# anton-galkovsky/pointcloudTraj

Measured on AMD Instinct MI355X. Metric: nn_queries_per_sec_10M_point_cloud, higher is better.
Workload: dtype f64; 1 GPU; C3-throughput: 10000000 uniform fp32 points in [0,100.0)^3 (seed 3), 1048576 uniform NN queries per step (4 distinct batches in rotation, seeds [5, 1005, 2005, 3005]), grid kernel, inputs resident in HBM; points_per_gpu=10000000, total_points=10000000, algo=grid, query_batches_in_rotation=4, gpu_work_before_the_warmup_steps=none, full=False, parallelism=single GPU, cards=1

## Files before the change

pointcloudtraj_amd/csrc/kernels.hpp:

```cpp
#pragma once
#include <hip/hip_runtime.h>
#include <stdint.h>
#include <type_traits>

#pragma clang fp contract(off)

#include "bernstein.hpp"
#include "scan.hpp"

namespace pct {

constexpr int kWave = 64;
constexpr uint32_t kNoIndex = 0xFFFFFFFFu;

__device__ __forceinline__ double dist2(double px, double py, double pz, double qx, double qy, double qz)
{
    double dx = px - qx, dy = py - qy, dz = pz - qz;
    double s = dx * dx;
    s = s + dy * dy;
    s = s + dz * dz;
    return s;
}

__device__ __forceinline__ bool better(double d2a, uint32_t ia, double d2b, uint32_t ib)
// ... 1025 lines not shown
}

__device__ __forceinline__ void coop_scan_exact(const float4 *__restrict__ pts, uint32_t s, uint32_t e, uint32_t sub, double qx,
                                                double qy, double qz, double &bd, uint32_t &bi)
{
    for (uint32_t p = s + sub; p < e; p += kCoop) {
        const float4 P = pts[p];
        const double d2 = dist2((double)P.x, (double)P.y, (double)P.z, qx, qy, qz);
        const uint32_t id = __float_as_uint(P.w);
        if (better(d2, id, bd, bi)) { bd = d2; bi = id; }
    }
}

template <bool COUNT>
__device__ __forceinline__ void coop_scan_cube_or_shell(const GridDesc &G, const float4 *__restrict__ pts,
                                                        const uint32_t *__restrict__ cell_start, int cx, int cy, int cz, int r,
                                                        bool full, uint32_t sub, double qx, double qy, double qz, double &bd,
                                                        uint32_t &bi, uint32_t &npts, uint32_t &nruns)
{
    const int x0 = max(cx - r, 0), x1 = min(cx + r, G.gx - 1);
    const int y0 = max(cy - r, 0), y1 = min(cy + r, G.gy - 1);
    const int z0 = max(cz - r, 0), z1 = min(cz + r, G.gz - 1);
    for (int zz = z0; zz <= z1; zz++) {
        const bool zface = (zz == cz - r) || (zz == cz + r);
        for (int yy = y0; yy <= y1; yy++) {
            const uint32_t row = cell_lin(G, 0, yy, zz);
            if (full || zface || yy == cy - r || yy == cy + r) {
                const uint32_t s = cell_start[row + x0], e = cell_start[row + x1 + 1];
                if (COUNT && sub == 0) { npts += e - s; nruns += 1; }
                coop_scan_exact(pts, s, e, sub, qx, qy, qz, bd, bi);
            } else {
                if (cx - r >= 0) {
                    const uint32_t s = cell_start[row + cx - r], e = cell_start[row + cx - r + 1];
                    if (COUNT && sub == 0) { npts += e - s; nruns += 1; }
                    coop_scan_exact(pts, s, e, sub, qx, qy, qz, bd, bi);
                }
                if (cx + r <= G.gx - 1) {
                    const uint32_t s = cell_start[row + cx + r], e = cell_start[row + cx + r + 1];
                    if (COUNT && sub == 0) { npts += e - s; nruns += 1; }
                    coop_scan_exact(pts, s, e, sub, qx, qy, qz, bd, bi);
                }
            }
        }
    }
}

template <int NR, int DEPTH, bool TAIL = false, bool NARROW = false>
__device__ __forceinline__ void coop_screen_rows(const float4 *__restrict__ pts, const uint32_t (&rs)[NR], const uint32_t (&re)[NR],
                                                 uint32_t sub, float qxf, float qyf, float qzf, double qx, double qy, double qz,
                                                 double &bd, uint32_t &bi)
{
    float m1 = __builtin_huge_valf(), m2 = __builtin_huge_valf();
    uint32_t p1 = 0;
    float4 P[NR][DEPTH];
#pragma unroll
    for (int k = 0; k < NR; k++) {
        const uint32_t a = rs[k], b = re[k];
        const uint32_t last = b - 1u;
#pragma unroll
        for (int j = 0; j < DEPTH; j++) P[k][j] = ld_at<NARROW>(pts, min(a + sub + kCoop * j, last));
    }
    uint32_t tp = 0;
    bool tail_on = false, tail_loops = false;
    float4 PT = make_float4(0.0f, 0.0f, 0.0f, 0.0f);
    if constexpr (TAIL) {
        constexpr uint32_t kMain = kCoop * DEPTH;
        uint32_t T = 0;
#pragma unroll
        for (int k = 0; k < NR; k++) {
            const uint32_t t = max(re[k] - rs[k], kMain) - kMain;
            tp = sub >= T ? rs[k] + kMain + (sub - T) : tp;
            T += t;
        }
        tail_on = sub < T && T <= (uint32_t)kCoop;
        tail_loops = T > (uint32_t)kCoop;
        const uint32_t a = rs[NR - 1], b = re[NR - 1];
        tp = tail_on ? tp : min(a + sub + kCoop * (DEPTH - 1), b - 1u);
        PT = ld_at<NARROW>(pts, tp);
    }
#pragma unroll
    for (int k = 0; k < NR; k++) {
        const uint32_t a = rs[k], b = re[k];
#pragma unroll
        for (int j = 0; j < DEPTH; j++) {
            const uint32_t p = a + sub + kCoop * j;
            const float dx = P[k][j].x - qxf, dy = P[k][j].y - qyf, dz = P[k][j].z - qzf;
            float d = __builtin_fmaf(dz, dz, __builtin_fmaf(dy, dy, dx * dx));
            d = (p < b) ? d : __builtin_huge_valf();
            const bool lt = d < m1;
            m2 = __builtin_amdgcn_fmed3f(m1, m2, d);
            p1 = lt ? p : p1;
            m1 = fminf(m1, d);
        }
    }
    auto long_row = [&](uint32_t a, uint32_t b) {
        for (uint32_t p = a + kCoop * DEPTH + sub; p < b; p += kCoop) {
            const float4 Pp = ld_at<NARROW>(pts, p);
            const float dx = Pp.x - qxf, dy = Pp.y - qyf, dz = Pp.z - qzf;
            const float d = __builtin_fmaf(dz, dz, __builtin_fmaf(dy, dy, dx * dx));
            const bool lt = d < m1;
            m2 = __builtin_amdgcn_fmed3f(m1, m2, d);
            p1 = lt ? p : p1;
            m1 = fminf(m1, d);
        }
    };
    if constexpr (TAIL) {
        const float dx = PT.x - qxf, dy = PT.y - qyf, dz = PT.z - qzf;
        float d = __builtin_fmaf(dz, dz, __builtin_fmaf(dy, dy, dx * dx));
        d = tail_on ? d : __builtin_huge_valf();
        const bool lt = d < m1;
        m2 = __builtin_amdgcn_fmed3f(m1, m2, d);
        p1 = lt ? tp : p1;
        m1 = fminf(m1, d);
        if (tail_loops) {
#pragma unroll
            for (int k = 0; k < NR; k++) long_row(rs[k], re[k]);
        }
    } else if constexpr (NR <= 4) {
#pragma unroll
        for (int k = 0; k < NR; k++) long_row(rs[k], re[k]);
    } else {
#pragma unroll 1
        for (int k = 0; k < NR; k++) long_row(rs[k], re[k]);
    }
    auto fold = [&](auto off) {
        constexpr int kPat = swz_xor(decltype(off)::value);
        const float o1 = swz_f32<kPat>(m1), o2 = swz_f32<kPat>(m2);
        const uint32_t op = swz_u32<kPat>(p1);
        const bool lt = o1 < m1;
        m2 = fminf(fminf(m2, o2), fmaxf(m1, o1));
        p1 = lt ? op : p1;
        m1 = fminf(m1, o1);
    };
    fold(std::integral_constant<int, 1>{});
    fold(std::integral_constant<int, 2>{});
    fold(std::integral_constant<int, 4>{});
    bd = __builtin_huge_val();
    bi = kNoIndex;
    if (m1 < __builtin_huge_valf() && m2 > m1 * (1.0f + 0x1p-19f) + 0x1p-90f) {
        const float4 W = ld_at<NARROW>(pts, p1);
        bd = dist2((double)W.x, (double)W.y, (double)W.z, qx, qy, qz);
        bi = __float_as_uint(W.w);
    } else {
#pragma unroll 1
        for (int k = 0; k < NR; k++) coop_scan_exact(pts, rs[k], re[k], sub, qx, qy, qz, bd, bi);
        coop_argmin8(bd, bi);
    }
}

template <bool COUNT>
__device__ __forceinline__ void coop_nn_search(const GridDesc &G, const float4 *__restrict__ pts,
                                               const uint32_t *__restrict__ cell_start, float qxf, float qyf, float qzf,
                                               uint32_t sub, double &bd, uint32_t &bi, uint32_t &npts, uint32_t &nruns)
{
    const double qx = (double)qxf, qy = (double)qyf, qz = (double)qzf;
    const int cx = cell_coord(qxf, G.ox, G.inv_h, G.gx);
    const int cy = cell_coord(qyf, G.oy, G.inv_h, G.gy);
    const int cz = cell_coord(qzf, G.oz, G.inv_h, G.gz);
    bd = __builtin_huge_val();
    bi = kNoIndex;
    if (G.octant_first) {
        const float fx = (qxf - G.ox) * G.inv_h - (float)cx, fy = (qyf - G.oy) * G.inv_h - (float)cy, fz = (qzf - G.oz) * G.inv_h - (float)cz;
        const int xa = max(fx < 0.5f ? cx - 1 : cx, 0), xb = min(fx < 0.5f ? cx : cx + 1, G.gx - 1);
        const int ya = max(fy < 0.5f ? cy - 1 : cy, 0), yb = min(fy < 0.5f ? cy : cy + 1, G.gy - 1);
        const int za = max(fz < 0.5f ? cz - 1 : cz, 0), zb = min(fz < 0.5f ? cz : cz + 1, G.gz - 1);
        uint32_t rs[4], re[4];
        {
            const int ri = (int)sub & 3;
            const bool ok = !((ri >> 1) && zb == za) && !((ri & 1) && yb == ya);
            const uint32_t row = cell_lin(G, 0, (ri & 1) ? yb : ya, (ri >> 1) ? zb : za);
            const uint32_t a = cell_start[row + xa], b = cell_start[row + xb + 1];
            const uint32_t my_s = a, my_e = ok ? b : a;
            if (COUNT && sub < 4) { npts += my_e - my_s; nruns += ok ? 1u : 0u; }
#pragma unroll
            for (int k = 0; k < 4; k++) { rs[k] = (uint32_t)__shfl((int)my_s, k, kCoop); re[k] = (uint32_t)__shfl((int)my_e, k, kCoop); }
        }
        coop_screen_rows<4, 2>(pts, rs, re, sub, qxf, qyf, qzf, qx, qy, qz, bd, bi);
        double bound = __builtin_huge_val();
        if (xa > 0) bound = fmin(bound, qx - (G.oxd + (double)xa * G.hd));
        if (xb < G.gx - 1) bound = fmin(bound, (G.oxd + (double)(xb + 1) * G.hd) - qx);
        if (ya > 0) bound = fmin(bound, qy - (G.oyd + (double)ya * G.hd));
        if (yb < G.gy - 1) bound = fmin(bound, (G.oyd + (double)(yb + 1) * G.hd) - qy);
        if (za > 0) bound = fmin(bound, qz - (G.ozd + (double)za * G.hd));
        if (zb < G.gz - 1) bound = fmin(bound, (G.ozd + (double)(zb + 1) * G.hd) - qz);
        if (bound == __builtin_huge_val()) return;
        bound -= G.hd * (1.0 / 256.0);
        if (bound > 0.0 && bd <= bound * bound) return;
    }
    {
        const int x0 = max(cx - 1, 0), x1 = min(cx + 1, G.gx - 1);
        uint32_t my_s = 0, my_e = 0, s8 = 0, e8 = 0;
        {
            const int zz = cz + (int)sub / 3 - 1, yy = cy + (int)sub % 3 - 1;
            const bool ok = zz >= 0 && zz < G.gz && yy >= 0 && yy < G.gy;
            const uint32_t row = ok ? cell_lin(G, 0, yy, zz) : 0u;
            const uint32_t a = cell_start[row + x0], b = cell_start[row + x1 + 1];
            my_s = a;
            my_e = ok ? b : a;
            const int z8 = cz + 1, y8 = cy + 1;
            const bool ok8 = z8 < G.gz && y8 < G.gy;
            const uint32_t row8 = ok8 ? cell_lin(G, 0, y8, z8) : 0u;
            const uint32_t a8 = cell_start[row8 + x0], b8 = cell_start[row8 + x1 + 1];
            s8 = a8;
            e8 = ok8 ? b8 : a8;
            if (COUNT && sub == 0) {
                npts += e8 - s8; nruns += ok8 ? 1u : 0u;
            }
            if (COUNT) {
                npts += my_e - my_s; nruns += ok ? 1u : 0u;
            }
        }
        uint32_t rs[9], re[9];
#pragma unroll
        for (int k = 0; k < 8; k++) { rs[k] = (uint32_t)__shfl((int)my_s, k, kCoop); re[k] = (uint32_t)__shfl((int)my_e, k, kCoop); }
        rs[8] = s8; re[8] = e8;

        coop_screen_rows<9, 1>(pts, rs, re, sub, qxf, qyf, qzf, qx, qy, qz, bd, bi);
    }
    for (int r = 1;; r++) {
        if (r > 1) {
            coop_scan_cube_or_shell<COUNT>(G, pts, cell_start, cx, cy, cz, r, false, sub, qx, qy, qz, bd, bi, npts, nruns);
            coop_argmin8(bd, bi);
        }
        const double bound = cube_bound(G, cx, cy, cz, r, qx, qy, qz);
        if (bound == __builtin_huge_val() || (bound > 0.0 && bd <= bound * bound)) break;
    }
}


__device__ __forceinline__ bool block_leaves_undecided(const GridDesc &G, int cx, int cy, int cz, int xa, int xb, int ya, int yb, int za, int zb,
                                                       float fx, float fy, float fz, double qx, double qy, double qz, double bd)
{
    {
        const float inf = __builtin_huge_valf();
        float bc = inf;
        bc = fminf(bc, xa > 0 ? fx + (float)(cx - xa) : inf);
        bc = fminf(bc, xb < G.gx - 1 ? (float)(xb + 1 - cx) - fx : inf);
        bc = fminf(bc, ya > 0 ? fy + (float)(cy - ya) : inf);
        bc = fminf(bc, yb < G.gy - 1 ? (float)(yb + 1 - cy) - fy : inf);
        bc = fminf(bc, za > 0 ? fz + (float)(cz - za) : inf);
        bc = fminf(bc, zb < G.gz - 1 ? (float)(zb + 1 - cz) - fz : inf);
        if (bc < inf && fmaxf(fmaxf(fabsf(fx), fabsf(fy)), fabsf(fz)) < 2.0f) {
            const double b = (double)((bc - 0.015625f) * (float)G.hd * 0.999999f);
            if (b > 0.0 && bd <= b * b) return false;
        }
    }
    double bound = __builtin_huge_val();
    if (xa > 0) bound = fmin(bound, qx - (G.oxd + (double)xa * G.hd));
    if (xb < G.gx - 1) bound = fmin(bound, (G.oxd + (double)(xb + 1) * G.hd) - qx);
    if (ya > 0) bound = fmin(bound, qy - (G.oyd + (double)ya * G.hd));
    if (yb < G.gy - 1) bound = fmin(bound, (G.oyd + (double)(yb + 1) * G.hd) - qy);
    if (za > 0) bound = fmin(bound, qz - (G.ozd + (double)za * G.hd));
    if (zb < G.gz - 1) bound = fmin(bound, (G.ozd + (double)(zb + 1) * G.hd) - qz);
    if (bound == __builtin_huge_val()) return false;
    bound -= G.hd * (1.0 / 256.0);
    return !(bound > 0.0 && bd <= bound * bound);
}

template <bool COUNT, bool NARROW>
__device__ __forceinline__ bool coop_stage0(const GridDesc &G, const float4 *__restrict__ pts, const uint32_t *__restrict__ cell_start,
                                            float qxf, float qyf, float qzf, uint32_t sub, double &bd, uint32_t &bi, uint32_t &npts,
                                            uint32_t &nruns)
{
    const double qx = (double)qxf, qy = (double)qyf, qz = (double)qzf;
    const int cx = cell_coord(qxf, G.ox, G.inv_h, G.gx);
    const int cy = cell_coord(qyf, G.oy, G.inv_h, G.gy);
    const int cz = cell_coord(qzf, G.oz, G.inv_h, G.gz);
    const float fx = (qxf - G.ox) * G.inv_h - (float)cx, fy = (qyf - G.oy) * G.inv_h - (float)cy, fz = (qzf - G.oz) * G.inv_h - (float)cz;
    const int xa = max(fx < 0.5f ? cx - 1 : cx, 0), xb = min(fx < 0.5f ? cx : cx + 1, G.gx - 1);
    const int ya = max(fy < 0.5f ? cy - 1 : cy, 0), yb = min(fy < 0.5f ? cy : cy + 1, G.gy - 1);
    const int za = max(fz < 0.5f ? cz - 1 : cz, 0), zb = min(fz < 0.5f ? cz : cz + 1, G.gz - 1);
    uint32_t rs[4], re[4];
    if (G.blocks) {
        const uint32_t u = (uint32_t)(fx < 0.5f ? cx : cx + 1), v = (uint32_t)(fy < 0.5f ? cy : cy + 1), w = (uint32_t)(fz < 0.5f ? cz : cz + 1);
        const uint4 *ent = G.blocks + 2u * ((w * ((uint32_t)G.gy + 1u) + v) * ((uint32_t)G.gx + 1u) + u);
        const uint4 S = ent[0], E = ent[1];
        rs[0] = S.x; rs[1] = S.y; rs[2] = S.z; rs[3] = S.w;
        re[0] = E.x; re[1] = E.y; re[2] = E.z; re[3] = E.w;
        if (COUNT && sub < 4) {
            const int ri = (int)sub;
            const bool ok = !((ri >> 1) && zb == za) && !((ri & 1) && yb == ya);
            npts += re[ri] - rs[ri]; nruns += ok ? 1u : 0u;
        }
    } else {
        const int ri = (int)sub & 3;
        const bool ok = !((ri >> 1) && zb == za) && !((ri & 1) && yb == ya);
        const uint32_t row = cell_lin(G, 0, (ri & 1) ? yb : ya, (ri >> 1) ? zb : za);
        const uint32_t a = ld_at<NARROW>(cell_start, row + (uint32_t)xa), b = ld_at<NARROW>(cell_start, row + (uint32_t)xb + 1u);
        const uint32_t my_s = a, my_e = ok ? b : a;
        if (COUNT && sub < 4) { npts += my_e - my_s; nruns += ok ? 1u : 0u; }
        rs[0] = swz_u32<swz_group_lane(0)>(my_s); re[0] = swz_u32<swz_group_lane(0)>(my_e);
        rs[1] = swz_u32<swz_group_lane(1)>(my_s); re[1] = swz_u32<swz_group_lane(1)>(my_e);
        rs[2] = swz_u32<swz_group_lane(2)>(my_s); re[2] = swz_u32<swz_group_lane(2)>(my_e);
        rs[3] = swz_u32<swz_group_lane(3)>(my_s); re[3] = swz_u32<swz_group_lane(3)>(my_e);
    }
    uint32_t pk0 = (uint32_t)xa | ((uint32_t)xb << 10) | ((uint32_t)ya << 20), pk1 = (uint32_t)yb | ((uint32_t)za << 10) | ((uint32_t)zb << 20);
    asm volatile("" : "+v"(pk0), "+v"(pk1));
    coop_screen_rows<4, 2, true, NARROW>(pts, rs, re, sub, qxf, qyf, qzf, qx, qy, qz, bd, bi);
    asm volatile("" : "+v"(pk0), "+v"(pk1));
    return block_leaves_undecided(G, cx, cy, cz, (int)(pk0 & 1023u), (int)((pk0 >> 10) & 1023u), (int)(pk0 >> 20), (int)(pk1 & 1023u),
                                  (int)((pk1 >> 10) & 1023u), (int)(pk1 >> 20), fx, fy, fz, qx, qy, qz, bd);
}

template <bool COUNT>
__device__ __forceinline__ void wave_cube_search(const GridDesc &G, const float4 *__restrict__ pts, const uint32_t *__restrict__ cell_start,
                                                 float qxf, float qyf, float qzf, double &bd, uint32_t &bi, uint32_t &npts, uint32_t &nruns)
{
    const uint32_t lane = threadIdx.x & 63;
    const double qx = (double)qxf, qy = (double)qyf, qz = (double)qzf;
    const int cx = cell_coord(qxf, G.ox, G.inv_h, G.gx);
    const int cy = cell_coord(qyf, G.oy, G.inv_h, G.gy);
    const int cz = cell_coord(qzf, G.oz, G.inv_h, G.gz);
    const int x0 = max(cx - 1, 0), x1 = min(cx + 1, G.gx - 1);
    uint32_t my_s, my_e;
    {
        const int l = lane < 9 ? (int)lane : 0;
        const int zz = cz + l / 3 - 1, yy = cy + l % 3 - 1;
        const bool ok = zz >= 0 && zz < G.gz && yy >= 0 && yy < G.gy;
        const uint32_t row = ok ? cell_lin(G, 0, yy, zz) : 0u;
        const uint32_t a = cell_start[row + x0], b = cell_start[row + x1 + 1];
        my_s = a;
        my_e = ok ? b : a;
        if (COUNT && lane < 9) { npts += my_e - my_s; nruns += ok ? 1u : 0u; }
    }
    uint32_t rs[9], re[9];
#pragma unroll
    for (int k = 0; k < 9; k++) {
        rs[k] = (uint32_t)__builtin_amdgcn_readlane((int)my_s, k);
        re[k] = (uint32_t)__builtin_amdgcn_readlane((int)my_e, k);
    }
    float m1 = __builtin_huge_valf(), m2 = __builtin_huge_valf();
    uint32_t p1 = 0;
    float4 P[9];
#pragma unroll
    for (int k = 0; k < 9; k++) {
        const uint32_t a = rs[k], b = re[k];
        P[k] = pts[min(a + lane, b > a ? b - 1 : 0u)];
    }
#pragma unroll
    for (int k = 0; k < 9; k++) {
        const uint32_t p = rs[k] + lane;
        const float dx = P[k].x - qxf, dy = P[k].y - qyf, dz = P[k].z - qzf;
        float d = __builtin_fmaf(dz, dz, __builtin_fmaf(dy, dy, dx * dx));
        d = (p < re[k]) ? d : __builtin_huge_valf();
        const bool lt = d < m1;
        m2 = lt ? m1 : fminf(m2, d);
        p1 = lt ? p : p1;
        m1 = fminf(m1, d);
    }
#pragma unroll 1
    for (int k = 0; k < 9; k++)
        for (uint32_t p = rs[k] + 64u + lane; p < re[k]; p += 64u) {
            const float4 Pp = pts[p];
            const float dx = Pp.x - qxf, dy = Pp.y - qyf, dz = Pp.z - qzf;
            const float d = __builtin_fmaf(dz, dz, __builtin_fmaf(dy, dy, dx * dx));
            const bool lt = d < m1;
            m2 = lt ? m1 : fminf(m2, d);
            p1 = lt ? p : p1;
            m1 = fminf(m1, d);
        }
#pragma unroll
    for (int off = 1; off < 64; off <<= 1) {
        const float o1 = __shfl_xor(m1, off, kWave), o2 = __shfl_xor(m2, off, kWave);
        const uint32_t op = (uint32_t)__shfl_xor((int)p1, off, kWave);
        const bool lt = o1 < m1;
        m2 = fminf(fminf(m2, o2), lt ? m1 : o1);
        p1 = lt ? op : p1;
        m1 = fminf(m1, o1);
    }
    bd = __builtin_huge_val();
    bi = kNoIndex;
    if (m1 < __builtin_huge_valf() && m2 > m1 * (1.0f + 0x1p-19f) + 0x1p-90f) {
        const float4 W = pts[p1];
        bd = dist2((double)W.x, (double)W.y, (double)W.z, qx, qy, qz);
        bi = __float_as_uint(W.w);
    } else {
#pragma unroll 1
        for (int k = 0; k < 9; k++)
            for (uint32_t p = rs[k] + lane; p < re[k]; p += 64u) {
                const float4 Pp = pts[p];
                const double d2 = dist2((double)Pp.x, (double)Pp.y, (double)Pp.z, qx, qy, qz);
                const uint32_t id = __float_as_uint(Pp.w);
                if (better(d2, id, bd, bi)) { bd = d2; bi = id; }
            }
        wave_argmin(bd, bi);
    }
}

template <bool COUNT>
__device__ __forceinline__ void coop_finish_shells(const GridDesc &G, const float4 *__restrict__ pts, const uint32_t *__restrict__ cell_start,
                                                   float qxf, float qyf, float qzf, uint32_t sub, double &bd, uint32_t &bi, uint32_t &npts,
                                                   uint32_t &nruns)
{
    const double qx = (double)qxf, qy = (double)qyf, qz = (double)qzf;
    const int cx = cell_coord(qxf, G.ox, G.inv_h, G.gx);
    const int cy = cell_coord(qyf, G.oy, G.inv_h, G.gy);
    const int cz = cell_coord(qzf, G.oz, G.inv_h, G.gz);
    for (int r = 1;; r++) {
        if (r > 1) {
            coop_scan_cube_or_shell<COUNT>(G, pts, cell_start, cx, cy, cz, r, false, sub, qx, qy, qz, bd, bi, npts, nruns);
            coop_argmin8(bd, bi);
        }
        const double bound = cube_bound(G, cx, cy, cz, r, qx, qy, qz);
        if (bound == __builtin_huge_val() || (bound > 0.0 && bd <= bound * bound)) break;
    }
}

template <bool COUNT, bool NARROW>
__device__ __forceinline__ void coop_wave_search(const GridDesc &G, const float4 *__restrict__ pts, const uint32_t *__restrict__ cell_start, bool live,
                                                 float qxf, float qyf, float qzf, uint32_t sub, double &bd, uint32_t &bi, uint32_t &npts, uint32_t &nruns)
{
    bd = __builtin_huge_val();
    bi = kNoIndex;
    bool undecided = false;
    if (live) undecided = coop_stage0<COUNT, NARROW>(G, pts, cell_start, qxf, qyf, qzf, sub, bd, bi, npts, nruns);
    unsigned long long todo = __builtin_amdgcn_ballot_w64(undecided && sub == 0);
    while (todo) {
        const int g = __builtin_ctzll(todo);
        todo &= todo - 1;
        const float bx = __uint_as_float((uint32_t)__builtin_amdgcn_readlane((int)__float_as_uint(qxf), g)),
                    by = __uint_as_float((uint32_t)__builtin_amdgcn_readlane((int)__float_as_uint(qyf), g)),
                    bz = __uint_as_float((uint32_t)__builtin_amdgcn_readlane((int)__float_as_uint(qzf), g));
        double cbd;
        uint32_t cbi;
        wave_cube_search<COUNT>(G, pts, cell_start, bx, by, bz, cbd, cbi, npts, nruns);
        if (((threadIdx.x & 63) >> 3) == (uint32_t)(g >> 3)) { bd = cbd; bi = cbi; }
    }
    if (live && undecided) coop_finish_shells<COUNT>(G, pts, cell_start, qxf, qyf, qzf, sub, bd, bi, npts, nruns);
}

template <bool COUNT, bool NARROW>
__global__ __launch_bounds__(256) __attribute__((amdgpu_waves_per_eu(7, 7))) void nn_grid_coop_kernel(GridDesc G, const float4 *__restrict__ pts,
                                                           const uint32_t *__restrict__ cell_start,
                                                           const float *__restrict__ q, uint32_t Q, uint32_t index_base,
                                                           const float4 *__restrict__ qsorted,
                                                           uint32_t *__restrict__ out_idx, double *__restrict__ out_d2,
                                                           WorkCounters *__restrict__ work)
{
    const uint32_t sub = threadIdx.x & (kCoop - 1);
    const uint32_t bslot = qsorted ? xcd_contiguous_block(blockIdx.x, gridDim.x) : blockIdx.x;
    const uint32_t slot = bslot * (256 / kCoop) + (threadIdx.x / kCoop);
    uint32_t npts = 0, nruns = 0;
    if (G.octant_first) {
        const bool live = slot < Q;
        uint32_t t = slot;
        float qxf = 0.0f, qyf = 0.0f, qzf = 0.0f;
        if (live) {
            if (qsorted) {
                const float4 R = ld_at<NARROW>(qsorted, slot);
                qxf = R.x; qyf = R.y; qzf = R.z; t = __float_as_uint(R.w);
            } else {
                qxf = q[3 * t]; qyf = q[3 * t + 1]; qzf = q[3 * t + 2];
            }
        }
        double bd;
        uint32_t bi;
        coop_wave_search<COUNT, NARROW>(G, pts, cell_start, live, qxf, qyf, qzf, sub, bd, bi, npts, nruns);
        if (live && sub == 0) {
            st_at<NARROW>(out_idx, t, reported_index(bd, bi, index_base));
            st_at<NARROW>(out_d2, t, bd);
        }
    } else if (slot < Q) {
        uint32_t t = slot;
        float qxf, qyf, qzf;
        if (qsorted) {
            const float4 R = qsorted[slot];
            qxf = R.x; qyf = R.y; qzf = R.z; t = __float_as_uint(R.w);
        } else {
            qxf = q[3 * t]; qyf = q[3 * t + 1]; qzf = q[3 * t + 2];
        }
        double bd;
        uint32_t bi;
        coop_nn_search<COUNT>(G, pts, cell_start, qxf, qyf, qzf, sub, bd, bi, npts, nruns);
        if (sub == 0) {
            out_idx[t] = reported_index(bd, bi, index_base);
            out_d2[t] = bd;
        }
    }
    if (COUNT) {
        unsigned long long a = npts, b = nruns;
#pragma unroll
        for (int off = 32; off > 0; off >>= 1) {
            a += (unsigned long long)__shfl_xor((long long)a, off, kWave);
            b += (unsigned long long)__shfl_xor((long long)b, off, kWave);
        }
        if ((threadIdx.x & 63) == 0) { WorkCounters *w = work + (blockIdx.x & (kWorkSlots - 1)); atomicAdd(&w->points, a); atomicAdd(&w->cells, b); }
    }
}

struct BallBox { int x0, x1, y0, y1, z0, z1; };

__device__ __forceinline__ void grid_ball_box(const GridDesc &G, float qxf, float qyf, float qzf, float rf, BallBox &B)
{
    const float pad0 = fabsf(rf) + 0.01f * (1.0f / G.inv_h);
    const float padx = pad0 + 0x1p-22f * (fabsf(qxf) + fabsf(rf)), pady = pad0 + 0x1p-22f * (fabsf(qyf) + fabsf(rf)),
                padz = pad0 + 0x1p-22f * (fabsf(qzf) + fabsf(rf));
    const float hx = qxf + padx, hy = qyf + pady, hz = qzf + padz;
    B.x0 = cell_coord(qxf - padx, G.ox, G.inv_h, G.gx); B.x1 = hx == hx ? cell_coord(hx, G.ox, G.inv_h, G.gx) : G.gx - 1;
    B.y0 = cell_coord(qyf - pady, G.oy, G.inv_h, G.gy); B.y1 = hy == hy ? cell_coord(hy, G.oy, G.inv_h, G.gy) : G.gy - 1;
    B.z0 = cell_coord(qzf - padz, G.oz, G.inv_h, G.gz); B.z1 = hz == hz ? cell_coord(hz, G.oz, G.inv_h, G.gz) : G.gz - 1;
}

template <bool COUNT>
__global__ __launch_bounds__(256) void count_grid_coop_kernel(GridDesc G, const float4 *__restrict__ pts,
                                                              const uint32_t *__restrict__ cell_start,
                                                              const float *__restrict__ q, const float *__restrict__ rad, uint32_t Q,
                                                              const float4 *__restrict__ qsorted, uint32_t *__restrict__ count,
                                                              WorkCounters *__restrict__ work)
{
    const uint32_t sub = threadIdx.x & (kCoop - 1);
    const uint32_t bslot = qsorted ? xcd_contiguous_block(blockIdx.x, gridDim.x) : blockIdx.x;
    const uint32_t slot = bslot * (256 / kCoop) + (threadIdx.x / kCoop);
    uint32_t npts = 0, nruns = 0;
    if (slot < Q) {
        uint32_t t = slot;
        float qxf, qyf, qzf;
        if (qsorted) {
            const float4 R = qsorted[slot];
            qxf = R.x; qyf = R.y; qzf = R.z; t = __float_as_uint(R.w);
        } else {
            qxf = q[3 * t]; qyf = q[3 * t + 1]; qzf = q[3 * t + 2];
        }
        const float rf = rad[t];
        const double qx = (double)qxf, qy = (double)qyf, qz = (double)qzf;
        const double r2 = (double)rf * (double)rf;
        BallBox B;
        grid_ball_box(G, qxf, qyf, qzf, rf, B);
        const int x0 = B.x0, x1 = B.x1, y0 = B.y0, z0 = B.z0;
        const int ny = B.y1 - y0 + 1, nrows = ny * (B.z1 - z0 + 1);
        uint32_t c = 0;
        for (int base = 0; base < nrows; base += 16) {
            uint32_t bs[2], be[2];
#pragma unroll
            for (int h = 0; h < 2; h++) {
                const int k = base + 8 * h + (int)sub;
                const bool ok = k < nrows;
                const uint32_t row = ok ? cell_lin(G, 0, y0 + k % ny, z0 + k / ny) : 0u;
                const uint32_t a = cell_start[row + x0], b = cell_start[row + x1 + 1];
                bs[h] = a; be[h] = ok ? b : a;
                if (COUNT) { npts += be[h] - bs[h]; nruns += ok ? 1u : 0u; }
            }
#pragma unroll
            for (int i = 0; i < 8; i++) {
                if (base + 2 * i >= nrows) break;
                uint32_t rs[2], re[2];
#pragma unroll
                for (int j = 0; j < 2; j++) {
                    const int r = 2 * i + j;
                    rs[j] = (uint32_t)__shfl((int)bs[r >> 3], r & 7, kCoop);
                    re[j] = (uint32_t)__shfl((int)be[r >> 3], r & 7, kCoop);
                }
                float4 P[2][4];
#pragma unroll
                for (int j = 0; j < 2; j++) {
                    const uint32_t last = re[j] > rs[j] ? re[j] - 1 : 0u;
#pragma unroll
                    for (int d = 0; d < 4; d++) P[j][d] = pts[min(rs[j] + sub + kCoop * d, last)];
                }
#pragma unroll
                for (int j = 0; j < 2; j++) {
#pragma unroll
                    for (int d = 0; d < 4; d++) {
                        const bool in = rs[j] + sub + kCoop * d < re[j];
                        c += (in && dist2((double)P[j][d].x, (double)P[j][d].y, (double)P[j][d].z, qx, qy, qz) <= r2) ? 1u : 0u;
                    }
                }
#pragma unroll 1
                for (int j = 0; j < 2; j++)
                    for (uint32_t p = rs[j] + 4 * kCoop + sub; p < re[j]; p += kCoop) {
                        const float4 Pp = pts[p];
                        c += dist2((double)Pp.x, (double)Pp.y, (double)Pp.z, qx, qy, qz) <= r2 ? 1u : 0u;
                    }
            }
        }
#pragma unroll
        for (int off = 1; off < kCoop; off <<= 1) c += (uint32_t)__shfl_xor((int)c, off, kWave);
        if (sub == 0) count[t] = c;
    }
    if (COUNT) {
        unsigned long long a = npts, b = nruns;
#pragma unroll
        for (int off = 32; off > 0; off >>= 1) {
            a += (unsigned long long)__shfl_xor((long long)a, off, kWave);
            b += (unsigned long long)__shfl_xor((long long)b, off, kWave);
        }
        if ((threadIdx.x & 63) == 0) { WorkCounters *w = work + (blockIdx.x & (kWorkSlots - 1)); atomicAdd(&w->points, a); atomicAdd(&w->cells, b); }
    }
}

struct ExpressOut { double d2; double radius; uint32_t idx; uint32_t count; };

struct ExpressSignal { uint32_t *counter; uint32_t *seq; uint32_t value; };

__device__ __forceinline__ void express_done(const ExpressSignal &S)
{
    if (!S.seq) return;
    __threadfence_system();
    bool last = gridDim.x == 1;
    if (!last) {
        last = atomicAdd(S.counter, 1u) == gridDim.x - 1;
        if (last) { atomicExch(S.counter, 0u); __threadfence_system(); }
    }
    if (last) __hip_atomic_store(S.seq, S.value, __ATOMIC_RELEASE, __HIP_MEMORY_SCOPE_SYSTEM);
}

__device__ __forceinline__ void express_done_block(const ExpressSignal &S)
{
    if (!S.seq) return;
    __threadfence_system();
    __syncthreads();
    if (threadIdx.x == 0) express_done(S);
}

__global__ __launch_bounds__(256) void import_floats_kernel(const float *__restrict__ h_src, uint32_t n, float *__restrict__ dst)
{
    const uint32_t i = blockIdx.x * blockDim.x + threadIdx.x;
    if (i < n) dst[i] = h_src[i];
}

__global__ __launch_bounds__(256) void export_results_kernel(const uint32_t *__restrict__ idx, const double *__restrict__ d2, uint32_t Q,
                                                             uint32_t *__restrict__ h_idx, double *__restrict__ h_d2, ExpressSignal sig)
{
    const uint32_t i = blockIdx.x * blockDim.x + threadIdx.x;
    if (i < Q) {
        h_idx[i] = idx[i];
        if (d2) h_d2[i] = d2[i];
    }
    express_done_block(sig);
}

__device__ __forceinline__ void tie_merge(double &d, uint32_t &i, uint32_t &c, double od, uint32_t oi, uint32_t oc)
{
    if (od < d) { d = od; i = oi; c = oc; }
    else if (od == d) { c += oc; i = min(i, oi); }
}

__global__ __launch_bounds__(1024) void nn_small_kernel(const float *__restrict__ x, const float *__restrict__ y,
                                                        const float *__restrict__ z, uint32_t n, double qx, double qy, double qz,
                                                        uint32_t index_base, ExpressOut *__restrict__ out, ExpressSignal sig)
{
    double bd = __builtin_huge_val();
    uint32_t bi = kNoIndex, bc = 0;
    for (uint32_t i = threadIdx.x; i < n; i += 1024) {
        const double d2 = dist2((double)x[i], (double)y[i], (double)z[i], qx, qy, qz);
        if (d2 < bd) { bd = d2; bi = i; bc = 1; }
        else if (d2 == bd) bc++;
    }
#pragma unroll
    for (int off = 32; off > 0; off >>= 1) {
        const double od = __shfl_xor(bd, off, kWave);
        const uint32_t oi = (uint32_t)__shfl_xor((int)bi, off, kWave), oc = (uint32_t)__shfl_xor((int)bc, off, kWave);
        tie_merge(bd, bi, bc, od, oi, oc);
    }
    __shared__ double s_d[16];
    __shared__ uint32_t s_i[16], s_c[16];
    if ((threadIdx.x & 63) == 0) { s_d[threadIdx.x >> 6] = bd; s_i[threadIdx.x >> 6] = bi; s_c[threadIdx.x >> 6] = bc; }
    __syncthreads();
    if (threadIdx.x == 0) {
        for (int w = 1; w < 16; w++) tie_merge(bd, bi, bc, s_d[w], s_i[w], s_c[w]);
        out->d2 = bd;
        out->idx = reported_index(bd, bi, index_base);
        out->count = bc;
        express_done(sig);
    }
}

__global__ __launch_bounds__(1024) void radius_small_kernel(const float *__restrict__ x, const float *__restrict__ y,
                                                            const float *__restrict__ z, uint32_t n, double qx, double qy, double qz,
                                                            double r2, uint32_t index_base, uint32_t *__restrict__ ids, uint32_t cap,
                                                            ExpressOut *__restrict__ out, ExpressSignal sig)
{
    __shared__ uint32_t s_n;
    if (threadIdx.x == 0) s_n = 0;
    __syncthreads();
    for (uint32_t i = threadIdx.x; i < n; i += 1024)
        if (dist2((double)x[i], (double)y[i], (double)z[i], qx, qy, qz) <= r2) {
            const uint32_t pos = atomicAdd(&s_n, 1u);
            if (pos < cap) ids[pos] = i + index_base;
        }
    __syncthreads();
    if (threadIdx.x == 0) out->count = s_n;
    express_done_block(sig);
}

__global__ __launch_bounds__(256) void nn_small_batch_kernel(const float *__restrict__ x, const float *__restrict__ y,
                                                             const float *__restrict__ z, uint32_t n,
                                                             const double *__restrict__ q, uint32_t index_base,
                                                             ExpressOut *__restrict__ out, ExpressSignal sig)
{
    __shared__ double s_d[4];
    __shared__ uint32_t s_i[4];
    const double qx = q[3 * blockIdx.x], qy = q[3 * blockIdx.x + 1], qz = q[3 * blockIdx.x + 2];
    double bd = __builtin_huge_val();
    uint32_t bi = kNoIndex;
    for (uint32_t i = threadIdx.x; i < n; i += 256) {
        const double d2 = dist2((double)x[i], (double)y[i], (double)z[i], qx, qy, qz);
        if (d2 < bd) { bd = d2; bi = i; }
    }
    wave_argmin(bd, bi);
    if ((threadIdx.x & 63) == 0) { s_d[threadIdx.x >> 6] = bd; s_i[threadIdx.x >> 6] = bi; }
    __syncthreads();
    if (threadIdx.x == 0) {
        for (int w = 1; w < 4; w++)
            if (better(s_d[w], s_i[w], bd, bi)) { bd = s_d[w]; bi = s_i[w]; }
        out[blockIdx.x].d2 = bd;
        out[blockIdx.x].idx = reported_index(bd, bi, index_base);
        express_done(sig);
    }
}

__global__ __launch_bounds__(256) void radius_small_batch_kernel(const float *__restrict__ x, const float *__restrict__ y,
                                                                 const float *__restrict__ z, uint32_t n,
                                                                 const double *__restrict__ q, const double *__restrict__ r,
                                                                 uint32_t index_base, uint32_t *__restrict__ ids,
                                                                 uint32_t cap_per_query, ExpressOut *__restrict__ out, ExpressSignal sig)
{
    __shared__ uint32_t s_n;
    if (threadIdx.x == 0) s_n = 0;
    __syncthreads();
    const double qx = q[3 * blockIdx.x], qy = q[3 * blockIdx.x + 1], qz = q[3 * blockIdx.x + 2];
    const double r2 = r[blockIdx.x] * r[blockIdx.x];
    for (uint32_t i = threadIdx.x; i < n; i += 256)
        if (dist2((double)x[i], (double)y[i], (double)z[i], qx, qy, qz) <= r2) {
            const uint32_t pos = atomicAdd(&s_n, 1u);
            if (pos < cap_per_query) ids[(size_t)blockIdx.x * cap_per_query + pos] = i + index_base;
        }
    __syncthreads();
    if (threadIdx.x == 0) out[blockIdx.x].count = s_n;
// ... 278 lines not shown
```

Before: 8.243 billion queries/s.

## Seed wave fallback with stage-0 result and scan only reachable remainder cells

```diff
diff --git a/pointcloudtraj_amd/csrc/kernels.hpp b/pointcloudtraj_amd/csrc/kernels.hpp
--- a/pointcloudtraj_amd/csrc/kernels.hpp
+++ b/pointcloudtraj_amd/csrc/kernels.hpp
@@ -1351,88 +1351,105 @@
                                   (int)((pk1 >> 10) & 1023u), (int)(pk1 >> 20), fx, fy, fz, qx, qy, qz, bd);
 }
 
+constexpr int kRemRows = 4;
 template <bool COUNT>
-__device__ __forceinline__ void wave_cube_search(const GridDesc &G, const float4 *__restrict__ pts, const uint32_t *__restrict__ cell_start,
-                                                 float qxf, float qyf, float qzf, double &bd, uint32_t &bi, uint32_t &npts, uint32_t &nruns)
+__device__ __forceinline__ void wave_remainder_search(const GridDesc &G, const float4 *__restrict__ pts, const uint32_t *__restrict__ cell_start,
+                                                      float qxf, float qyf, float qzf, double &bd, uint32_t &bi, uint32_t &npts, uint32_t &nruns)
 {
     const uint32_t lane = threadIdx.x & 63;
     const double qx = (double)qxf, qy = (double)qyf, qz = (double)qzf;
     const int cx = cell_coord(qxf, G.ox, G.inv_h, G.gx);
     const int cy = cell_coord(qyf, G.oy, G.inv_h, G.gy);
     const int cz = cell_coord(qzf, G.oz, G.inv_h, G.gz);
-    const int x0 = max(cx - 1, 0), x1 = min(cx + 1, G.gx - 1);
-    uint32_t my_s, my_e;
+    const float fx = (qxf - G.ox) * G.inv_h - (float)cx, fy = (qyf - G.oy) * G.inv_h - (float)cy, fz = (qzf - G.oz) * G.inv_h - (float)cz;
+    const int xa = max(fx < 0.5f ? cx - 1 : cx, 0), xb = min(fx < 0.5f ? cx : cx + 1, G.gx - 1);
+    const int ya = max(fy < 0.5f ? cy - 1 : cy, 0), yb = min(fy < 0.5f ? cy : cy + 1, G.gy - 1);
+    const int za = max(fz < 0.5f ? cz - 1 : cz, 0), zb = min(fz < 0.5f ? cz : cz + 1, G.gz - 1);
+    auto gap = [&](int c, int g, double o, double q) {
+        const double ninf = -__builtin_huge_val();
+        const double below = c > 0 ? (o + (double)c * G.hd) - q : ninf;
+        const double above = c < g - 1 ? q - (o + (double)(c + 1) * G.hd) : ninf;
+        return fmax(fmax(below, above) - G.hd * (1.0 / 256.0), 0.0);
+    };
+    uint32_t my_s = 0, my_e = 0;
     {
         const int l = lane < 9 ? (int)lane : 0;
         const int zz = cz + l / 3 - 1, yy = cy + l % 3 - 1;
-        const bool ok = zz >= 0 && zz < G.gz && yy >= 0 && yy < G.gy;
-        const uint32_t row = ok ? cell_lin(G, 0, yy, zz) : 0u;
-        const uint32_t a = cell_start[row + x0], b = cell_start[row + x1 + 1];
-        my_s = a;
-        my_e = ok ? b : a;
-        if (COUNT && lane < 9) { npts += my_e - my_s; nruns += ok ? 1u : 0u; }
-    }
-    uint32_t rs[9], re[9];
-#pragma unroll
-    for (int k = 0; k < 9; k++) {
-        rs[k] = (uint32_t)__builtin_amdgcn_readlane((int)my_s, k);
-        re[k] = (uint32_t)__builtin_amdgcn_readlane((int)my_e, k);
-    }
-    float m1 = __builtin_huge_valf(), m2 = __builtin_huge_valf();
-    uint32_t p1 = 0;
-    float4 P[9];
-#pragma unroll
-    for (int k = 0; k < 9; k++) {
-        const uint32_t a = rs[k], b = re[k];
-        P[k] = pts[min(a + lane, b > a ? b - 1 : 0u)];
-    }
-#pragma unroll
-    for (int k = 0; k < 9; k++) {
-        const uint32_t p = rs[k] + lane;
-        const float dx = P[k].x - qxf, dy = P[k].y - qyf, dz = P[k].z - qzf;
-        float d = __builtin_fmaf(dz, dz, __builtin_fmaf(dy, dy, dx * dx));
-        d = (p < re[k]) ? d : __builtin_huge_valf();
-        const bool lt = d < m1;
-        m2 = lt ? m1 : fminf(m2, d);
-        p1 = lt ? p : p1;
-        m1 = fminf(m1, d);
-    }
-#pragma unroll 1
-    for (int k = 0; k < 9; k++)
-        for (uint32_t p = rs[k] + 64u + lane; p < re[k]; p += 64u) {
-            const float4 Pp = pts[p];
-            const float dx = Pp.x - qxf, dy = Pp.y - qyf, dz = Pp.z - qzf;
-            const float d = __builtin_fmaf(dz, dz, __builtin_fmaf(dy, dy, dx * dx));
-            const bool lt = d < m1;
-            m2 = lt ? m1 : fminf(m2, d);
-            p1 = lt ? p : p1;
-            m1 = fminf(m1, d);
-        }
-#pragma unroll
-    for (int off = 1; off < 64; off <<= 1) {
-        const float o1 = __shfl_xor(m1, off, kWave), o2 = __shfl_xor(m2, off, kWave);
-        const uint32_t op = (uint32_t)__shfl_xor((int)p1, off, kWave);
-        const bool lt = o1 < m1;
-        m2 = fminf(fminf(m2, o2), lt ? m1 : o1);
-        p1 = lt ? op : p1;
-        m1 = fminf(m1, o1);
-    }
-    bd = __builtin_huge_val();
-    bi = kNoIndex;
-    if (m1 < __builtin_huge_valf() && m2 > m1 * (1.0f + 0x1p-19f) + 0x1p-90f) {
-        const float4 W = pts[p1];
-        bd = dist2((double)W.x, (double)W.y, (double)W.z, qx, qy, qz);
-        bi = __float_as_uint(W.w);
-    } else {
-#pragma unroll 1
-        for (int k = 0; k < 9; k++)
-            for (uint32_t p = rs[k] + lane; p < re[k]; p += 64u) {
-                const float4 Pp = pts[p];
-                const double d2 = dist2((double)Pp.x, (double)Pp.y, (double)Pp.z, qx, qy, qz);
-                const uint32_t id = __float_as_uint(Pp.w);
-                if (better(d2, id, bd, bi)) { bd = d2; bi = id; }
+        const bool ok = lane < 9 && zz >= 0 && zz < G.gz && yy >= 0 && yy < G.gy;
+        const bool block_row = yy >= ya && yy <= yb && zz >= za && zz <= zb;
+        const double gy = gap(yy, G.gy, G.oyd, qy), gz = gap(zz, G.gz, G.ozd, qz);
+        auto reach = [&](int c) {
+            const bool valid = ok && c >= 0 && c <= G.gx - 1 && !(block_row && c >= xa && c <= xb);
+            const double gxx = gap(c, G.gx, G.oxd, qx);
+            return valid & !(((gxx * gxx + gy * gy) + gz * gz) * (1.0 - 0x1p-40) > bd);
+        };
+        const bool rm = reach(cx - 1), r0 = reach(cx), rp = reach(cx + 1);
+        if (rm || r0 || rp) {
+            const int lo = rm ? cx - 1 : (r0 ? cx : cx + 1), hi = rp ? cx + 1 : (r0 ? cx : cx - 1);
+            const uint32_t row = cell_lin(G, 0, yy, zz);
+            my_s = cell_start[row + (uint32_t)lo];
+            my_e = cell_start[row + (uint32_t)hi + 1u];
+            if (COUNT) { npts += my_e - my_s; nruns += 1u; }
+        }
+    }
+    float thr = (float)bd;
+    if ((double)thr < bd) thr = __uint_as_float(__float_as_uint(thr) + 1u);
+    thr = thr * (1.0f + 0x1p-19f) + 0x1p-90f;
+    double ld = bd;
+    uint32_t li = bi;
+    auto exact = [&](const float4 &R) {
+        float sx = qxf, sy = qyf, sz = qzf;
+        asm volatile("" : "+s"(sx), "+s"(sy), "+s"(sz));
+        const double d2 = dist2((double)R.x, (double)R.y, (double)R.z, (double)sx, (double)sy, (double)sz);
+        const uint32_t id = __float_as_uint(R.w);
+        if (better(d2, id, ld, li)) { ld = d2; li = id; }
+    };
+    bool any = false;
+    unsigned long long rows = __builtin_amdgcn_ballot_w64(my_e > my_s);
+    while (rows) {
+        uint32_t rs[kRemRows], len[kRemRows];
+#pragma unroll
+        for (int j = 0; j < kRemRows; j++) {
+            rs[j] = 0; len[j] = 0;
+            if (rows) {
+                const int k = __builtin_ctzll(rows);
+                rows &= rows - 1;
+                rs[j] = (uint32_t)__builtin_amdgcn_readlane((int)my_s, k);
+                len[j] = (uint32_t)__builtin_amdgcn_readlane((int)my_e, k) - rs[j];
             }
-        wave_argmin(bd, bi);
+        }
+        float4 P[kRemRows];
+#pragma unroll
+        for (int j = 0; j < kRemRows; j++)
+            if (len[j]) P[j] = pts[rs[j] + min(lane, len[j] - 1u)];
+        uint32_t cm = 0;
+#pragma unroll
+        for (int j = 0; j < kRemRows; j++)
+            if (len[j]) {
+                const float dx = P[j].x - qxf, dy = P[j].y - qyf, dz = P[j].z - qzf;
+                const float d = __builtin_fmaf(dz, dz, __builtin_fmaf(dy, dy, dx * dx));
+                cm |= (uint32_t)((lane < len[j]) & (d <= thr)) << j;
+            }
+#pragma unroll
+        for (int j = 0; j < kRemRows; j++)
+            if (len[j] > 64u)
+                for (uint32_t o = 64u + lane; o < len[j]; o += 64u) {
+                    const float4 R = pts[rs[j] + o];
+                    const float dx = R.x - qxf, dy = R.y - qyf, dz = R.z - qzf;
+                    const float d = __builtin_fmaf(dz, dz, __builtin_fmaf(dy, dy, dx * dx));
+                    if (d <= thr) { exact(R); cm |= 1u << kRemRows; }
+                }
+        if (__builtin_amdgcn_ballot_w64(cm != 0u)) {
+            any = true;
+#pragma unroll
+            for (int j = 0; j < kRemRows; j++)
+                if ((cm >> j) & 1u) exact(P[j]);
+        }
+    }
+    if (any) {
+        wave_argmin(ld, li);
+        bd = ld;
+        bi = li;
     }
 }
 
@@ -1470,9 +1487,9 @@
         const float bx = __uint_as_float((uint32_t)__builtin_amdgcn_readlane((int)__float_as_uint(qxf), g)),
                     by = __uint_as_float((uint32_t)__builtin_amdgcn_readlane((int)__float_as_uint(qyf), g)),
                     bz = __uint_as_float((uint32_t)__builtin_amdgcn_readlane((int)__float_as_uint(qzf), g));
-        double cbd;
-        uint32_t cbi;
-        wave_cube_search<COUNT>(G, pts, cell_start, bx, by, bz, cbd, cbi, npts, nruns);
+        double cbd = __hiloint2double(__builtin_amdgcn_readlane(__double2hiint(bd), g), __builtin_amdgcn_readlane(__double2loint(bd), g));
+        uint32_t cbi = (uint32_t)__builtin_amdgcn_readlane((int)bi, g);
+        wave_remainder_search<COUNT>(G, pts, cell_start, bx, by, bz, cbd, cbi, npts, nruns);
         if (((threadIdx.x & 63) >> 3) == (uint32_t)(g >> 3)) { bd = cbd; bi = cbi; }
     }
     if (live && undecided) coop_finish_shells<COUNT>(G, pts, cell_start, qxf, qyf, qzf, sub, bd, bi, npts, nruns);
```

Result: faster. 8.536 billion queries/s (median of 6 runs) (+3.5%).
